# woolgathering/pyPeriod

Measured on AMD Instinct MI355X. Metric: window-projections/sec (all-p sweep, N=4096), higher is better.
Workload: dtype f64

## Files before the change

### include/periodhip.h

```cpp
#ifndef PERIODHIP_H
#define PERIODHIP_H

#include <stdint.h>

#ifdef __cplusplus
extern "C" {
#endif

#define PH_VERSION 100

#define PH_OK 0
#define PH_E_ARG (-1)
#define PH_E_HIP (-2)
#define PH_E_NOMEM (-3)
#define PH_E_CAP (-4)
#define PH_E_UNSUPPORTED (-5)

#define PH_F64 0
#define PH_F32 1

#define PH_FLAG_TRUNC 1u
#define PH_FLAG_ORTH 2u
#define PH_FLAG_SINGLE 4u
#define PH_FLAG_DEVICE 8u
// ... 9 lines not shown
#define PH_ST_NO_PERIOD 1
#define PH_ST_ITER_CAP 2
#define PH_ST_CAP 3

typedef struct ph_ctx ph_ctx;

int ph_version(void);
const char* ph_last_error(void);
int ph_device_count(int* count);
int ph_create(int device, ph_ctx** out);
int ph_destroy(ph_ctx* ctx);
#define PH_STREAM_DEFAULT ((void*)1)
int ph_set_stream(ph_ctx* ctx, void* hip_stream);
int ph_sync(ph_ctx* ctx);
int ph_timer_begin(ph_ctx* ctx);
int ph_timer_end(ph_ctx* ctx, float* elapsed_ms);
int ph_profile_enable(ph_ctx* ctx, int on);
int ph_profile_read(ph_ctx* ctx, float* ms, int cap, int* count);
const char* ph_profile_name(ph_ctx* ctx, int i);
int ph_device_info(ph_ctx* ctx, int* num_cu, int* lds_bytes);
int ph_max_window(ph_ctx* ctx, int dtype, unsigned flags, int* max_n);

int ph_sweep_plan_info(ph_ctx* ctx, int p_lo, int p_hi, int* n_pass, int* n_periods);

int ph_m_best_info(ph_ctx* ctx, int dtype, int N, int num, int min_length, int max_length, unsigned flags,
                   int* windows_per_workgroup, int* lds_bytes_per_sample);

int ph_m_best_plan_info(ph_ctx* ctx, int dtype, int N, int num, int min_length, int max_length, unsigned flags,
                        int* n_pass, int* n_periods);

int ph_m_best_screen_info(ph_ctx* ctx, int dtype, int N, int num, int min_length, int max_length, unsigned flags,
                          int gamma, int* n_entries, int* n_screened, long long* lds_elements);

int ph_periodic_norm(ph_ctx* ctx, const void* x, int dtype, int64_t W, int N, int p,
                     unsigned flags, double* out);

int ph_project_batch(ph_ctx* ctx, const void* x, int dtype, int64_t W, int N,
                     const int32_t* p_list, int n_p,
                     const int32_t* orth_off, const int32_t* orth_q, int table_max_p,
                     unsigned flags, void* out);

int ph_sweep(ph_ctx* ctx, const void* x, int dtype, int64_t W, int N, int p_lo, int p_hi,
             int mode, const int32_t* orth_off, const int32_t* orth_q, int table_max_p,
             unsigned flags, double* out);

int ph_m_best(ph_ctx* ctx, const void* x, int dtype, int64_t W, int N, int num,
// ... 136 lines not shown
```

### pyperiod_amd/_ffi.py

```python

from __future__ import annotations

import ctypes as C
import os

_HERE = os.path.dirname(os.path.abspath(__file__))
LIB_NAME = "libperiod_hip.so"
LIB_PATH = os.environ.get("PYPERIOD_AMD_LIB") or os.path.join(_HERE, LIB_NAME)

PH_OK, PH_E_ARG, PH_E_HIP, PH_E_NOMEM, PH_E_CAP, PH_E_UNSUPPORTED = 0, -1, -2, -3, -4, -5
PH_F64, PH_F32 = 0, 1
PH_FLAG_TRUNC, PH_FLAG_ORTH, PH_FLAG_SINGLE, PH_FLAG_DEVICE, PH_FLAG_NOSYNC = 1, 2, 4, 8, 16
PH_FLAG_KEEP_WEIGHTS = 32
PH_FLAG_OLA_NORM = 64
PH_STREAM_DEFAULT = 1
PH_SWEEP_NORM, PH_SWEEP_NORM_GAMMA, PH_SWEEP_MAXABS = 0, 1, 2
PH_ST_OK, PH_ST_NO_PERIOD, PH_ST_ITER_CAP, PH_ST_CAP = 0, 1, 2, 3
PH_QO_LDS_OVERLAY, PH_QO_LDS_BEHIND, PH_QO_HBM = 0, 1, 2
(PH_OP_PROJECT, PH_OP_SWEEP, PH_OP_M_BEST, PH_OP_SMALL_TO_LARGE, PH_OP_BEST_CORRELATION, PH_OP_BEST_FREQUENCY,
 PH_OP_RAMANUJAN, PH_OP_ORTH_POWERS, PH_OP_FOLD_SUMS, PH_OP_QO_FIT, PH_OP_QO_FIT_WIN, PH_OP_QO_ORTH_SELECT,
 PH_OP_QO_GET_PERIODS) = range(13)
PH_PLAN_KERNELS, PH_PLAN_K0, PH_PLAN_K1, PH_PLAN_STRIDE, PH_PLAN_LEN = 0, 1, 9, 8, 17
(PH_PLAN_VARIANT, PH_PLAN_WINDOW, PH_PLAN_SECOND, PH_PLAN_BLOCK, PH_PLAN_LDS_BYTES, PH_PLAN_SMALL_MEANS, PH_PLAN_WAVES,
 PH_PLAN_PAD) = range(8)
PH_PLAN_ONE, PH_PLAN_PAIR, PH_PLAN_FFT, PH_PLAN_CHIRP, PH_PLAN_DIRECT = 0, 1, 2, 3, 4
PH_PLAN_NONE, PH_PLAN_LDS, PH_PLAN_HBM = 0, 1, 2

_vp, _i, _i64, _u, _d = C.c_void_p, C.c_int, C.c_int64, C.c_uint, C.c_double
_pi32 = C.c_void_p

SIGNATURES = {
    "ph_version": [],
    "ph_device_count": [C.POINTER(_i)],
    "ph_create": [_i, C.POINTER(_vp)],
    "ph_destroy": [_vp],
    "ph_set_stream": [_vp, _vp],
    "ph_sync": [_vp],
    "ph_timer_begin": [_vp],
    "ph_timer_end": [_vp, C.POINTER(C.c_float)],
    "ph_device_info": [_vp, C.POINTER(_i), C.POINTER(_i)],
    "ph_max_window": [_vp, _i, _u, C.POINTER(_i)],
    "ph_sweep_plan_info": [_vp, _i, _i, C.POINTER(_i), C.POINTER(_i)],
    "ph_m_best_info": [_vp, _i, _i, _i, _i, _i, _u, C.POINTER(_i), C.POINTER(_i)],
    "ph_m_best_plan_info": [_vp, _i, _i, _i, _i, _i, _u, C.POINTER(_i), C.POINTER(_i)],
    "ph_m_best_screen_info": [_vp, _i, _i, _i, _i, _i, _u, _i, C.POINTER(_i), C.POINTER(_i), C.POINTER(C.c_longlong)],
    "ph_periodic_norm": [_vp, _vp, _i, _i64, _i, _i, _u, _vp],
    "ph_project_batch": [_vp, _vp, _i, _i64, _i, _pi32, _i, _pi32, _pi32, _i, _u, _vp],
    "ph_sweep": [_vp, _vp, _i, _i64, _i, _i, _i, _i, _pi32, _pi32, _i, _u, _vp],
    "ph_m_best": [_vp, _vp, _i, _i64, _i, _i, _i, _i, _i, _pi32, _pi32, _pi32, _pi32, _i, _u, _vp, _vp, _vp, _vp, _vp],
    "ph_profile_enable": [_vp, _i],
    "ph_profile_read": [_vp, C.POINTER(C.c_float), _i, C.POINTER(_i)],
    "ph_small_to_large": [_vp, _vp, _i, _i64, _i, _d, _i, _pi32, _pi32, _i, _u, _i, _vp, _vp, _vp, _vp, _vp],
    "ph_best_correlation": [_vp, _vp, _i, _i64, _i, _i, _i, _d, _pi32, _pi32, _i, _u, _vp, _vp, _vp, _vp],
    "ph_best_frequency": [_vp, _vp, _i, _i64, _i, _i, _i, _pi32, _pi32, _i, _u, _vp, _vp, _vp, _vp],
    "ph_ramanujan_norms": [_vp, _vp, _i, _i64, _i, _i, _i, _u, _vp],
    "ph_dict_project": [_vp, _vp, _vp, _i, _i, _u, _vp],
    "ph_qo_find_periods": [_vp, _vp, _i, _i64, _i, _i, _d, _i, _i, _i, _u, _vp, _vp, _vp, _vp, _vp, _vp, _vp],
    "ph_qo_greedy_win": [_vp, _vp, _i, _i64, _i, _vp, _i, _d, _i, _i, _i, _u, _vp, _vp, _vp, _vp, _vp, _vp, _vp],
    "ph_qo_fit": [_vp, _vp, _i, _i64, _i, _pi32, _pi32, _i, _i, _i, _i, _u, _vp, _vp, _vp, _vp],
    "ph_qo_fit_win": [_vp, _vp, _i, _i64, _i, _vp, _pi32, _pi32, _i, _i, _i, _i, _u, _vp, _vp, _vp, _vp],
    "ph_ramanujan_fit": [_vp, _vp, _i, _i64, _i, _i, _i, _d, _i, _i, _u, _vp, _vp, _vp, _vp, _vp, _vp, _vp],
    "ph_qo_feasible": [_vp, _i, _i, _i, _i, C.POINTER(_i)],
    "ph_qo_plan_info": [_vp, _i, _i, _i, _i, _u, C.POINTER(_i), C.POINTER(_i)],
    "ph_plan_info": [_vp, _i, _i, _i, _pi32, _i, _u, _pi32],
    "ph_orth_powers": [_vp, _vp, _i, _i64, _i, _i, _i, _u, _vp, _vp, _vp],
# ... 78 lines not shown
```

### pyperiod_amd/csrc/period_hip.hip

```cpp
#include <hip/hip_runtime.h>

#include <algorithm>
#include <cstdarg>
#include <cstdio>
#include <cstdlib>
#include <cstring>
#include <string>
#include <vector>

#include "../../include/periodhip.h"
#include "ph_kernels.h"
#include "ph_fit.h"
#include "ph_frames.h"

namespace {

thread_local std::string g_err;

int fail(int code, const char* fmt, ...) {
  char buf[512];
  va_list ap;
  va_start(ap, fmt);
  vsnprintf(buf, sizeof buf, fmt, ap);
  va_end(ap);
// ... 22 lines not shown

struct TableSlot {
  DevBuf dev;
  std::vector<int32_t> host;
  bool valid = false;
};

enum { T_PLIST, T_ORTH_OFF, T_ORTH_Q, T_FAC_OFF, T_FAC_Q, T_AUX0, T_AUX1, T_AUX2, T_AUX3, T_FIT_PHI, T_FIT_OFF, T_FIT_DQ, T_COUNT };
enum { B_IN, B_OUT0, B_OUT1, B_OUT2, B_OUT3, B_OUT4, B_WS0, B_WS1, B_GEN0, B_GBUF, B_GWIN, B_COUNT };

}

struct ph_ctx {
  int device = 0;
  hipStream_t own_stream = nullptr;
  hipStream_t stream = nullptr;
  hipEvent_t ev0 = nullptr, ev1 = nullptr;
  int num_cu = 0;
  int lds_limit = 0;
  DevBuf buf[B_COUNT];
  TableSlot tab[T_COUNT];
  DevBuf geom;
  DevBuf geomf;
  DevBuf kapf;
  int geom_n = -1, geom_max_p = -1;
  bool step1_pair = true;
  bool s2l_pair = true;
  bool bc_pair = true;
  bool pair_chain = true;
  bool pair_cover = true;
  bool pair_duo = true;
  DevBuf twid;
  int twid_len = -1;
  DevBuf bs_tab;
  int bs_L = -1, bs_M0 = -1;
  DevBuf plan;
  int plan_lo = -1, plan_hi = -1, plan_n = 0, plan_m = -1, plan_duo_n = 0;
  int plan_max_m = 4;
  int sweep_block = ph::kBlockWide;
  int step1_block = 0;
  int qo_block = 1024;
  int s2l_block = 1024;
  bool qo_hbm_window = false;
  bool hbm_window = false;
  int mob_max_p = -1;
  std::vector<int32_t> mob_off, mob_d, mob_mu;
// ... 110 lines not shown
  if (chains) max_m += 16;
  if (c->plan.p && c->plan_lo == p_lo && c->plan_hi == p_hi && c->plan_m == max_m && c->plan_duo_n == duo_n) {
    *out = static_cast<const ph::PassPlan*>(c->plan.p);
    *n_pass = c->plan_n;
    return PH_OK;
  }
  const std::vector<ph::PassPlan> host = build_plan(p_lo, p_hi, max_m & 7, mixed, chains, duo_n);
  PH_HIP(hipStreamSynchronize(c->stream));
  PH_TRY(ensure(c, c->plan, std::max<size_t>(1, host.size()) * sizeof(ph::PassPlan)));
  if (!host.empty())
    PH_HIP(hipMemcpyAsync(c->plan.p, host.data(), host.size() * sizeof(ph::PassPlan), hipMemcpyHostToDevice,
                          c->stream));
  PH_HIP(hipStreamSynchronize(c->stream));
  c->plan_lo = p_lo;
  c->plan_hi = p_hi;
  c->plan_m = max_m;
  c->plan_duo_n = duo_n;
  c->plan_n = (int)host.size();
  *out = static_cast<const ph::PassPlan*>(c->plan.p);
  *n_pass = c->plan_n;
  return PH_OK;
}

int prepare_geom(ph_ctx* c, int N, int max_p, const ph::PGeom** out) {
  if (c->geom.p && c->geom_n == N && c->geom_max_p >= max_p) {
    *out = static_cast<const ph::PGeom*>(c->geom.p);
    return PH_OK;
  }
  std::vector<ph::PGeom> host((size_t)max_p + 1);
  host[0] = ph::PGeom{0, 0, 0.0, 0.0};
  for (int p = 1; p <= max_p; ++p) {
    const int rows = (N + p - 1) / p;
    const int shortn = rows * p - N;
    host[p] = ph::PGeom{rows, p - shortn, 1.0 / rows, rows > 1 ? 1.0 / (rows - 1) : 0.0};
  }
  PH_HIP(hipStreamSynchronize(c->stream));
  PH_TRY(ensure(c, c->geom, host.size() * sizeof(ph::PGeom)));
  PH_HIP(hipMemcpyAsync(c->geom.p, host.data(), host.size() * sizeof(ph::PGeom), hipMemcpyHostToDevice, c->stream));
  std::vector<ph::PGeomF> hostf(host.size());
  for (size_t p = 0; p < host.size(); ++p)
    hostf[p] = ph::PGeomF{host[p].rows, host[p].nfull, (float)host[p].w_full, (float)host[p].w_short};
  PH_TRY(ensure(c, c->geomf, hostf.size() * sizeof(ph::PGeomF)));
  PH_HIP(hipMemcpyAsync(c->geomf.p, hostf.data(), hostf.size() * sizeof(ph::PGeomF), hipMemcpyHostToDevice, c->stream));
  std::vector<float> hostk(host.size(), 0.0f);
  for (size_t p = 1; p < host.size(); ++p) {
    const double k = ph::s2l_kappa(N, host[p].rows, (int)p);
    float f = (float)k;
    if ((double)f < k) f = std::nextafterf(f, INFINITY);
    hostk[p] = f;
  }
  PH_TRY(ensure(c, c->kapf, hostk.size() * sizeof(float)));
  PH_HIP(hipMemcpyAsync(c->kapf.p, hostk.data(), hostk.size() * sizeof(float), hipMemcpyHostToDevice, c->stream));
  PH_HIP(hipStreamSynchronize(c->stream));
  c->geom_n = N;
  c->geom_max_p = max_p;
  *out = static_cast<const ph::PGeom*>(c->geom.p);
  return PH_OK;
}

int check_common(ph_ctx* c, const void* x, int dtype, int64_t W, int N) {
  if (!c) return fail(PH_E_ARG, "ctx is NULL");
  if (!x) return fail(PH_E_ARG, "x is NULL");
  if (dtype != PH_F64 && dtype != PH_F32) return fail(PH_E_ARG, "dtype must be PH_F64 or PH_F32");
  if (W < 1 || W > 0x7fffffffLL / 64) return fail(PH_E_ARG, "W=%lld out of range", (long long)W);
  if (N < 1) return fail(PH_E_ARG, "N=%d must be >= 1", N);
  return PH_OK;
// ... 628 lines not shown
    if (v >= 64 && v <= 1024 && v % 64 == 0) c->qo_block = v;
  }
  if (std::getenv("PH_QO_HBM_WINDOW")) c->qo_hbm_window = true;
  if (const char* e = std::getenv("PH_HBM_WINDOW"))
    if (std::atoi(e) != 0) c->hbm_window = c->qo_hbm_window = true;
  if (const char* e = std::getenv("PH_SWEEP_BLOCK")) {
    const int v = std::atoi(e);
    if (v >= 64 && v <= 512 && v % 64 == 0) c->sweep_block = v;
  }
  *out = c;
  return PH_OK;
}

int ph_destroy(ph_ctx* c) {
  if (!c) return PH_OK;
  (void)hipSetDevice(c->device);
  (void)hipStreamSynchronize(c->stream);
  for (DevBuf& b : c->buf)
    if (b.p) (void)hipFree(b.p);
  for (TableSlot& t : c->tab)
    if (t.dev.p) (void)hipFree(t.dev.p);
  if (c->geom.p) (void)hipFree(c->geom.p);
  if (c->geomf.p) (void)hipFree(c->geomf.p);
  if (c->kapf.p) (void)hipFree(c->kapf.p);
  if (c->plan.p) (void)hipFree(c->plan.p);
  if (c->twid.p) (void)hipFree(c->twid.p);
  if (c->bs_tab.p) (void)hipFree(c->bs_tab.p);
  for (hipEvent_t e : c->prof_ev) (void)hipEventDestroy(e);
  if (c->ev0) (void)hipEventDestroy(c->ev0);
  if (c->ev1) (void)hipEventDestroy(c->ev1);
  if (c->own_stream) (void)hipStreamDestroy(c->own_stream);
  delete c;
  return PH_OK;
}

int ph_set_stream(ph_ctx* c, void* hip_stream) {
  if (!c) return fail(PH_E_ARG, "ctx is NULL");
  const hipError_t e = hipStreamSynchronize(c->stream);
  if (hip_stream == PH_STREAM_DEFAULT)
    c->stream = nullptr;
  else
    c->stream = hip_stream ? static_cast<hipStream_t>(hip_stream) : c->own_stream;
  if (e != hipSuccess) {
    (void)hipGetLastError();
    return fail(PH_E_HIP, "ph_set_stream: draining the previous stream failed (%s); the new stream is bound",
                hipGetErrorString(e));
  }
  return PH_OK;
}

int ph_sweep_plan_info(ph_ctx* c, int p_lo, int p_hi, int* n_pass, int* n_periods) {
  if (!c || !n_pass || !n_periods) return fail(PH_E_ARG, "NULL argument");
  if (p_lo < 1 || p_hi < p_lo) return fail(PH_E_ARG, "need 1 <= p_lo <= p_hi (got %d, %d)", p_lo, p_hi);
  *n_pass = (int)build_plan(p_lo, p_hi, c->plan_max_m, true, c->pair_chain).size();
  *n_periods = p_hi - p_lo + 1;
  return PH_OK;
}

int ph_m_best_info(ph_ctx* c, int dtype, int N, int num, int min_length, int max_length, unsigned flags,
                   int* windows_per_workgroup, int* lds_bytes_per_sample) {
  if (!c || !windows_per_workgroup || !lds_bytes_per_sample) return fail(PH_E_ARG, "NULL argument");
  if (dtype != PH_F64 && dtype != PH_F32) return fail(PH_E_ARG, "dtype must be PH_F64 or PH_F32");
  if (max_length < 0) max_length = N / 3;
  const bool pair = pair_eligible(c, dtype, N, num, min_length, max_length, flags);
  *windows_per_workgroup = pair ? 2 : 1;
  *lds_bytes_per_sample = pair ? 8 : (int)elem_size(dtype);
  return PH_OK;
}

int ph_m_best_plan_info(ph_ctx* c, int dtype, int N, int num, int min_length, int max_length, unsigned flags, int* n_pass,
                        int* n_periods) {
  if (!c || !n_pass || !n_periods) return fail(PH_E_ARG, "NULL argument");
  if (dtype != PH_F64 && dtype != PH_F32) return fail(PH_E_ARG, "dtype must be PH_F64 or PH_F32");
  if (max_length < 0) max_length = N / 3;
  if (min_length < 1 || max_length < min_length)
    return fail(PH_E_ARG, "need 1 <= min_length <= max_length (got %d, %d)", min_length, max_length);
  const bool pair = pair_eligible(c, dtype, N, num, min_length, max_length, flags);
  const int p_scr = pair ? pair_screen_lo(c, min_length, max_length, 0) : min_length;
// ... 352 lines not shown
  PH_TRY(st.in(x, (size_t)W * N * sz, &dx));
  PH_TRY(st.out(B_OUT0, periods, (size_t)W * num * sizeof(uint32_t), &dper));
  PH_TRY(st.out(B_OUT1, powers, (size_t)W * num * sizeof(double), &dpow));
  PH_TRY(st.out(B_OUT2, bases, (size_t)W * num * N * sz, &dbases));
  PH_TRY(st.out(B_OUT3, status, (size_t)W * sizeof(int32_t), &dstat));
  void* dsweeps;
  PH_TRY(st.out(B_OUT4, n_sweeps, (size_t)W * sizeof(int32_t), &dsweeps));
  PH_TRY(ensure(c, c->buf[B_WS0], (size_t)W * sizeof(double)));
  double* dnorm = static_cast<double*>(c->buf[B_WS0].p);
  const int row_stride = (max_length + 127) & ~127;
  PH_TRY(ensure(c, c->buf[B_WS1], (size_t)W * num * row_stride * sz));
  void* drows = c->buf[B_WS1].p;
  const unsigned kflags = flags & (PH_FLAG_TRUNC | PH_FLAG_ORTH);
  const int max_iters = 12 * (P + num) + 64;
  const dim3 grid((unsigned)W);
  if (pair) {
    const size_t gstride = ph::win_stride((size_t)N);
    PH_TRY(ensure(c, c->buf[B_GWIN], (size_t)W * gstride * sizeof(double)));
    auto kernel = ph::k_mbest_step1_pair;
    PH_TRY(allow_lds(kernel, s1.lds));
    ProfScope ps_(c, "k_mbest_step1");
    hipLaunchKernelGGL(kernel, dim3((unsigned)((W + 1) / 2)), dim3(s1.block), s1.lds, c->stream, (const double*)dx, (int)W, N,
                       num, min_length, max_length, p_scr, gamma, tb.fac_off, tb.fac_q, geom,
                       static_cast<const ph::PGeomF*>(c->geomf.p), plan, n_pass,
                       static_cast<double*>(c->buf[B_GWIN].p), max_iters, (uint32_t*)dper, (double*)dpow, (double*)drows,
                       row_stride, dnorm, (int*)dstat, (int*)dsweeps);
  } else
  PH_TRY(dispatch(dtype, !gwin1, [&](auto t, auto lw) {
    using T = decltype(t);
    auto kernel = ph::k_mbest_step1<T, decltype(lw)::value>;
    PH_TRY(allow_lds(kernel, s1.lds));
    ProfScope ps_(c, "k_mbest_step1");
    hipLaunchKernelGGL(kernel, grid, dim3(s1.block), s1.lds, c->stream, (const T*)dx, N, num, min_length,
                       max_length, gamma, kflags, tb, geom, plan, n_pass, (T*)gbuf1, (T*)gwin1, max_iters,
                       (uint32_t*)dper, (double*)dpow, (T*)drows, row_stride, dnorm, (int*)dstat, (int*)dsweeps, s1.small_means);
    return (int)PH_OK;
  }));
  PH_TRY(launch_check("k_mbest_step1"));
  PH_TRY(dispatch(dtype, !gwin2, [&](auto t, auto lw) {
    using T = decltype(t);
    auto kernel = ph::k_mbest_step2<T, decltype(lw)::value>;
    PH_TRY(allow_lds(kernel, s2.lds));
    ProfScope ps_(c, "k_mbest_step2");
    hipLaunchKernelGGL(kernel, grid, dim3(s2.block), s2.lds, c->stream, N, num, gamma,
                       max_length, kflags, tb, geom,
                       max_fac, (T*)gbuf2, (T*)gwin2, (uint32_t*)dper, (double*)dpow, (T*)dbases, dnorm,
                       (const int*)dstat, (T*)drows, row_stride);
// ... 1135 lines not shown
```

### pyperiod_amd/csrc/ph_device.h

```cpp
#pragma once

#include <hip/hip_runtime.h>
#include <stdint.h>

namespace ph {

constexpr int kWave = 64;
constexpr int kBlock = 256;
constexpr int kBlockWide = 512;
constexpr int kMaxWaves = 16;

constexpr unsigned kTrunc = 1u;
constexpr unsigned kOrth = 2u;
constexpr unsigned kSingle = 4u;

struct Tables {
  const int* orth_off;
  const int* orth_q;
  const int* fac_off;
  const int* fac_q;
};

typedef volatile __attribute__((address_space(3))) int* lds_int_ptr;

// ... 121 lines not shown

__device__ __forceinline__ double block_max(double v, double* red) {
  const int tid = threadIdx.x;
  const int nw = (blockDim.x + kWave - 1) / kWave;
  v = wave_max(v);
  if ((tid & (kWave - 1)) == 0) red[tid >> 6] = v;
  __syncthreads();
  const double t = red_combine<true>(red, nw);
  __syncthreads();
  return uniform_f64(t);
}

struct Fold {
  int p;
  int rows;
  int nfull;
  int trows;
  __device__ __forceinline__ Fold(int N, int p_) : p(p_) {
    rows = (N + p_ - 1) / p_;
    const int shortn = rows * p_ - N;
    nfull = p_ - shortn;
    trows = shortn == 0 ? rows : rows - 1;
  }
  __device__ __forceinline__ int count(int j) const { return j < nfull ? rows : rows - 1; }
};

template <typename T>
__device__ __forceinline__ T column_sum(const T* __restrict__ xs, int j, int p, int n) {
  if (n <= 0) return T(0);
  const T* ptr = xs + j;
  T s = ptr[0];
  ptr += p;
  int r = 1;
  for (; r + 8 <= n; r += 8) {
    T v[8];
#pragma unroll
    for (int u = 0; u < 8; ++u) v[u] = ptr[u * p];
#pragma unroll
    for (int u = 0; u < 8; ++u) s += v[u];
    ptr += 8 * p;
  }
  for (; r < n; ++r) {
    s += ptr[0];
    ptr += p;
  }
  return s;
// ... 720 lines not shown
```

### pyperiod_amd/csrc/ph_kernels.h

```cpp
#pragma once

#include <type_traits>

#include "ph_device.h"
#include "ph_pair.h"

namespace ph {

struct Carve {
  unsigned char* base;
  size_t off;
  __device__ explicit Carve(unsigned char* b) : base(b), off(0) {}
  template <typename U>
  __device__ U* take(size_t n) {
    U* p = reinterpret_cast<U*>(base + off);
    off += (n * sizeof(U) + 15) & ~size_t(15);
    return p;
  }
};

__host__ __device__ inline size_t carve_bytes(size_t n, size_t elem) { return (n * elem + 15) & ~size_t(15); }

__host__ __device__ inline size_t win_stride(size_t len) { return (len + 3) & ~size_t(3); }

// ... 322 lines not shown
__device__ __forceinline__ double pair_pick_scale(double rsq, int N) {
  if (!pair_usable(rsq)) return 1.0;
  int e;
  (void)frexp(rsq / (double)N, &e);
  return ldexp(1.0, -(e >> 1));
}

__device__ __forceinline__ int pair_rows_upper(float fn, int q) {
  return (int)(fn * __builtin_amdgcn_rcpf((float)q) * 1.000001f) + 1;
}

__device__ __forceinline__ double pair_exact_part(const double* __restrict__ xs, int p, const PGeom& g, int first, int stride) {
  double part = 0.0;
  for (int j = first; j < p; j += stride) {
    const bool full = j < g.nfull;
    const double s = column_sum(xs, j, p, full ? g.rows : g.rows - 1);
    part = fma(s * s, full ? g.w_full : g.w_short, part);
  }
  return part;
}

__global__ __launch_bounds__(1024) __attribute__((amdgpu_waves_per_eu(PH_STEP1_WAVES, 8))) void k_mbest_step1_pair(
    const double* __restrict__ x, int W, int N, int num, int p_lo, int p_hi, int p_scr, int gamma,
    const int* __restrict__ fac_off, const int* __restrict__ fac_q, const PGeom* __restrict__ geom, const PGeomF* __restrict__ geomf, const PassPlan* __restrict__ plan, int n_pass,
    double* __restrict__ gres, int max_iters, uint32_t* __restrict__ periods_out, double* __restrict__ norms_out,
    double* __restrict__ rows_out, int row_stride, double* __restrict__ dnorm_out, int* __restrict__ status_out,
    int* __restrict__ sweeps_out) {
  extern __shared__ __attribute__((aligned(16))) unsigned char smem[];
  Carve cv(smem);
  f2* pw = cv.take<f2>(N + kPad);
  double* stg = cv.take<double>(N + kPad);
  double* red = cv.take<double>(kRedDoubles);
  double* wbest = cv.take<double>(kMaxWaves);
  int* wbestp = cv.take<int>(kMaxWaves);
  double* norms = cv.take<double>(2 * num);
  uint32_t* periods = cv.take<uint32_t>(2 * num);
  const int P = p_hi - p_lo + 1;
  const int SK = (P + 31) / 32;
  uint32_t* skip = cv.take<uint32_t>(2 * SK);
  int* list = cv.take<int>(2 * kPairListCap);
  int* ctl = cv.take<int>(16);
  double* dst2 = cv.take<double>(4);
  double* msm = cv.take<double>(kPairSmallP);
  double* prt = cv.take<double>(kPairSplitW);

  const int tid = threadIdx.x;
  const int wv = __builtin_amdgcn_readfirstlane(tid >> 6);
// ... 27 lines not shown
      dst2[w] = rsq * sc * sc * (1.0 + 1e-9);
      dst2[2 + w] = sc;
      ctl[10 + w] = exists ? 1 : 0;
      ctl[12 + w] = pair_usable(rsq) ? 0 : 1;
      if (exists) dnorm_out[gw] = periodic_norm_from_sq_n(rsq, sqrtN, 0);
    }
  }
#ifdef PH_PAIR_TIMERS
#ifndef PH_PAIR_TIMERS_WGS
#define PH_PAIR_TIMERS_WGS 6
#endif
  long long ts[5] = {0, 0, 0, 0, 0};
  long long ts0 = wall_clock64();
  int nsurv_tot = 0, nall = 0;
#define PH_PAIR_MARK(k)                     \
  {                                         \
    const long long now_ = wall_clock64();  \
    ts[k] += now_ - ts0;                    \
    ts0 = now_;                             \
  }
#else
#define PH_PAIR_MARK(k)
#endif
  const float fn = (float)N;
#ifdef PH_CLOCKS
  const long long ck0 = clock64(), wk0 = wall_clock64();
#endif
  for (;;) {
    __syncthreads();
    const bool act0 = __builtin_amdgcn_readfirstlane(ctl[10]) != 0, act1 = __builtin_amdgcn_readfirstlane(ctl[11]) != 0;
    if (!act0 && !act1) break;
    prio_by_progress(__builtin_amdgcn_readfirstlane(max(ctl[8], ctl[9])));
    if (wv == 0 && pair_lane() == 0) ctl[0] = ctl[1] = 0;
    f2* vals = reinterpret_cast<f2*>(stg);
    pair_sweep_plan<false, true>(
        pw, N, geomf, plan, wv, n_pass, nw, [&](float z, int q) { pair_store1(vals, z, q, p_lo); },
        [&](float z, int q_a, int q_b) { pair_store2(vals, z, q_a, q_b, p_lo); },
        PH_PAIR_QUEUE ? &ctl[14] : nullptr);
    __syncthreads();
    PH_PAIR_MARK(0)
    prio_short_phase();
    {
    const int tid = (wv << 6) + pair_lane();
    const int lane = tid & (kWave - 1);
    if (tid == 0) ctl[14] = nw;
    {
      const bool scr0 = act0 && !__builtin_amdgcn_readfirstlane(ctl[12]), scr1 = act1 && !__builtin_amdgcn_readfirstlane(ctl[13]);
      if (scr0 || scr1) {
        const double unit0 = uniform_f64(dst2[0]), unit1 = uniform_f64(dst2[1]);
        const int i0 = p_scr - p_lo;
        const bool cover = i0 > 0;
        const int SD = (i0 + 31) >> 5;
        uint32_t* seen = reinterpret_cast<uint32_t*>(stg);
        for (int k = tid; k < 2 * SD; k += blockDim.x) seen[k] = 0u;
        const double slack = cover ? pair_cover_slack(N) : 0.0;
        double lo0 = -1.0 / 0.0, lo1 = -1.0 / 0.0;
        for (int idx = i0 + tid; idx < P; idx += blockDim.x) {
          const int q = p_lo + idx;
          const f2 v = vals[idx];
          const double rad = pair_radius(pair_rows_upper(fn, q), q);
          const uint32_t bit = 1u << (idx & 31);
          double a = (double)v.x - rad * unit0, b = (double)v.y - rad * unit1;
          if (gamma) {
            const double rq = 1.0 / (double)q;
            a *= rq;
            b *= rq;
          }
          if (!(skip[idx >> 5] & bit) && a > lo0) lo0 = a;
          if (!(skip[SK + (idx >> 5)] & bit) && b > lo1) lo1 = b;
        }
        lo0 = wave_max(lo0);
        lo1 = wave_max(lo1);
        if (lane == 0) {
          red[wv] = lo0;
          red[kMaxWaves + wv] = lo1;
        }
        __syncthreads();
        lo0 = uniform_f64(red_combine<true>(red, nw));
        lo1 = uniform_f64(red_combine<true>(red + kMaxWaves, nw));
        const bool none0 = cover && scr0 && !(lo0 > -1.0 / 0.0), none1 = cover && scr1 && !(lo1 > -1.0 / 0.0);
        if (tid == 0 && none0) ctl[0] = kPairListCap + 1;
        if (tid == 0 && none1) ctl[1] = kPairListCap + 1;
        const double thr0 = lo0 - fabs(lo0) * 1e-9, thr1 = lo1 - fabs(lo1) * 1e-9;
        for (int idx = i0 + tid; idx < P; idx += blockDim.x) {
          const int q = p_lo + idx;
          const f2 v = vals[idx];
          const double rad = pair_radius(pair_rows_upper(fn, q), q) + slack;
          const uint32_t bit = 1u << (idx & 31);
          double a = (double)v.x + rad * unit0, b = (double)v.y + rad * unit1;
          if (gamma) {
            const double rq = 1.0 / (double)q;
            a *= rq;
            b *= rq;
          }
          const bool hit0 = scr0 && !none0 && a >= thr0, hit1 = scr1 && !none1 && b >= thr1;
          if (hit0 && !(skip[idx >> 5] & bit)) {
            const int k = atomicAdd(&ctl[0], 1);
            if (k < kPairListCap) list[k] = q;
          }
          if (hit1 && !(skip[SK + (idx >> 5)] & bit)) {
            const int k = atomicAdd(&ctl[1], 1);
            if (k < kPairListCap) list[kPairListCap + k] = q;
          }
          if (cover && (hit0 || hit1)) {
            const int f1 = fac_off[q + 1];
            for (int f = fac_off[q] - (p_lo == 1 ? 1 : 0); f < f1; ++f) {
              const int d = f < fac_off[q] ? 1 : fac_q[f];
              if (d < p_lo || d >= p_scr) continue;
              const int di = d - p_lo;
              const uint32_t dbit = 1u << (di & 31);
              for (int w = 0; w < 2; ++w) {
                if (!(w ? hit1 : hit0) || (skip[w * SK + (di >> 5)] & dbit)) continue;
                if (atomicOr(&seen[w * SD + (di >> 5)], dbit) & dbit) continue;
                const int k = atomicAdd(&ctl[w], 1);
                if (k < kPairListCap) list[w * kPairListCap + k] = d;
              }
            }
          }
        }
      }
    }
    __syncthreads();
    PH_PAIR_MARK(1)
// ... 88 lines not shown
        } else {
          for (int k = wv; k < ncand; k += nw) {
            const int p = exact_all ? p_lo + k : lst[k];
            if ((sk[(p - p_lo) >> 5] >> ((p - p_lo) & 31)) & 1u) continue;
            const PGeom g = geom[p];
            const double part = p < 64 ? wave_partial_small(stg, N, p, g, lane) : pair_exact_part(stg, p, g, lane, kWave);
            consider(wave_sum(part), p);
          }
          best = bestp != 0 ? periodic_norm_from_sq_n(best_ss, sqrtN, gamma ? bestp : 0) : 0.0;
          if (!(best > 0.0)) bestp = 0;
          if (lane == 0) {
            wbest[wv] = best;
            wbestp[wv] = bestp;
          }
          __syncthreads();
          red_argmax(wbest, wbestp, nw, best, bestp);
          __syncthreads();
        }
        PH_PAIR_MARK(3)
        if (bestp == 0) {
          status = 1;
        } else {
          int row = -1;
          for (int k = 0; k < num; ++k)
            if (per[k] == (uint32_t)bestp) row = k;
          int action;
          __syncthreads();
          if (row >= 0 && repeats < 10) {
            action = 2;
            if (tid == 0) nrm[row] += best;
            repeats += 1;
          } else if (row >= 0) {
            action = 0;
            if (tid == 0) sk[(bestp - p_lo) >> 5] |= 1u << ((bestp - p_lo) & 31);
            repeats = 0;
          } else {
            action = 1;
            row = filled;
            if (tid == 0) {
              per[row] = (uint32_t)bestp;
              nrm[row] = best;
            }
            filled += 1;
            repeats = 0;
          }
          double* brow = rows_out + (gw * (int64_t)num + (row < 0 ? 0 : row)) * row_stride;
          const bool more = filled < num;
          const double sc = uniform_f64(dst2[2 + w]);
          double* dst = gres + gw * gstride;
          double acc = 0.0;
          const Fold f(N, bestp);
          if (bestp <= kPairSmallP) {
            split_row_means(stg, msm, prt, N, bestp, tid, kPairSplitW);
            if (tid < bestp) {
              const double m = msm[tid];
              if (action == 1)
                brow[tid] = m;
              else if (action == 2)
                brow[tid] += m;
            }
            if (more) {
              int idx = tid % bestp;
              const int step = blockDim.x % bestp;
              for (int n = tid; n < N; n += blockDim.x) {
                const double v = stg[n] - msm[idx];
                dst[n] = v;
                pwf[2 * n + w] = (float)(v * sc);
                acc = fma(v, v, acc);
                idx += step;
                idx = idx >= bestp ? idx - bestp : idx;
              }
            }
          } else {
            for (int j = tid; j < bestp; j += blockDim.x) {
// ... 2395 lines not shown
```

### pyperiod_amd/csrc/ph_pair.h

```cpp
#pragma once

#include "ph_device.h"

namespace ph {

typedef float f2 __attribute__((ext_vector_type(2)));
typedef const volatile __attribute__((address_space(3))) f2* pair_ptr;

struct PGeomF {
  int rows;
  int nfull;
  float w_full;
  float w_short;
};

__device__ __forceinline__ f2 f2_make(float a, float b) {
  f2 r;
  r.x = a;
  r.y = b;
  return r;
}
__device__ __forceinline__ f2 f2_zero() { return f2_make(0.0f, 0.0f); }
__device__ __forceinline__ f2 f2_fma(f2 a, f2 b, f2 c) { return __builtin_elementwise_fma(a, b, c); }
__device__ __forceinline__ f2 f2_max(f2 a, f2 b) { return __builtin_elementwise_max(a, b); }
// ... 241 lines not shown
      "v_pk_fma_f32 %[acc], %[v], %[v], %[acc]\n\t"
      "s_mov_b64 exec, %[keep]"
      : [acc] "+v"(acc), [keep] "=&s"(keep)
      : [v] "v"(v), [m] "s"(lanes)
      : "scc");
}
__device__ __forceinline__ void f2_sq_acc_cut(f2& sa, f2& pa, f2& sb, f2& pb, f2 t, f2 d, unsigned long below, unsigned long inq) {
  unsigned long keep;
  asm volatile(
      "s_and_saveexec_b64 %[keep], %[below]\n\t"
      "v_pk_fma_f32 %[sa], %[t], %[t], %[sa]\n\t"
      "v_pk_fma_f32 %[pa], %[d], %[d], %[pa]\n\t"
      "s_andn2_b64 exec, %[keep], %[below]\n\t"
      "v_pk_fma_f32 %[pb], %[d], %[d], %[pb]\n\t"
      "s_and_b64 exec, exec, %[inq]\n\t"
      "v_pk_fma_f32 %[sb], %[t], %[t], %[sb]\n\t"
      "s_mov_b64 exec, %[keep]"
      : [sa] "+v"(sa), [pa] "+v"(pa), [sb] "+v"(sb), [pb] "+v"(pb), [keep] "=&s"(keep)
      : [t] "v"(t), [d] "v"(d), [below] "s"(below), [inq] "s"(inq)
      : "scc");
}

template <int R, int NR, int U, int PRO>
__device__ __forceinline__ void pair_duo_group(pair_ptr ptr, int q, int c, f2 (&pend)[R - 1], f2& sa, f2& pa, f2& sb, f2& pb) {
  static_assert(NR == R || NR == R - 1, "all rows (in front of the cut), or all but the last (behind it)");
  static_assert(PRO >= -1 && PRO <= U, "columns without a square are columns of the group");
  f2 v[NR][U];
#pragma unroll
  for (int r = 0; r < NR; ++r)
#pragma unroll
    for (int u = 0; u < U; ++u) v[r][u] = ptr[r * q + 64 * u];
  __builtin_amdgcn_s_waitcnt(0xC07F);
  __builtin_amdgcn_sched_barrier(0);
#pragma unroll
  for (int u = 0; u < U; ++u) {
    f2 t = v[0][u];
#pragma unroll
    for (int r = 1; r < NR; ++r) t += v[r][u];
    if (NR == R) sa = f2_fma(t, t, sa);
    else sb = f2_fma(t, t, sb);
    if (u >= PRO) {
      f2 d = pend[R - 2];
      if (NR == R) d += v[NR - 1][u];
      if (PRO < 0) d *= scalar_select_lt(c + u, R - 1, 0.0f, 1.0f);
      if (NR == R) pa = f2_fma(d, d, pa);
      else pb = f2_fma(d, d, pb);
    }
#pragma unroll
    for (int k = R - 2; k >= 1; --k) pend[k] = pend[k - 1] + v[k][u];
    pend[0] = v[0][u];
  }
}

template <int R, int NR>
__device__ __forceinline__ void pair_duo_edge(pair_ptr ptr, int q, unsigned long below, unsigned long inq, f2 (&pend)[R - 1],
                                              f2& sa, f2& pa, f2& sb, f2& pb) {
  static_assert(NR == R || NR == R - 1, "all rows (in front of the cut), or all but the last (behind it)");
  f2 v[NR];
#pragma unroll
  for (int r = 0; r < NR; ++r) v[r] = ptr[r * q];
  __builtin_amdgcn_s_waitcnt(0xC07F);
  __builtin_amdgcn_sched_barrier(0);
  f2 t = v[0];
#pragma unroll
  for (int r = 1; r < NR; ++r) t += v[r];
  f2 d = pend[R - 2];
  if (NR == R) d += v[NR - 1];
// ... 8 lines not shown
  pend[0] = v[0];
}

template <int R, int T0, int T1>
__device__ __forceinline__ void pair_duo_tail(const f2* __restrict__ xs, int q, int ncb, f2 (&pend)[R - 1], f2& pb) {
  const pair_ptr at = pair_at(xs) + 64 * ncb;
  f2 v[R - 1][R - 1];
#pragma unroll
  for (int t = T0; t < T1; ++t)
#pragma unroll
    for (int r = t; r < R - 1; ++r) v[r][t] = at[r * q + 64 * t];
  __builtin_amdgcn_s_waitcnt(0xC07F);
  __builtin_amdgcn_sched_barrier(0);
#pragma unroll
  for (int t = T0; t < T1; ++t) {
    pb = f2_fma(pend[R - 2], pend[R - 2], pb);
#pragma unroll
    for (int k = R - 2; k >= 1; --k) pend[k] = k >= t ? pend[k - 1] + v[k][t] : pend[k - 1];
    if (t == 0) pend[0] = v[0][0];
  }
  if (T1 == R - 1) f2_sq_acc_lanes(pb, pend[R - 2], pair_lanes_below(q - 64 * (ncb - 1)));
}

template <int R>
__device__ __forceinline__ void pair_duo_rows(const f2* __restrict__ xs, int N, int q, const PGeomF g, f2& base, f2& partner) {
  constexpr int UA = R <= 4 ? 4 : 2, UB = R <= 4 ? 4 : R == 5 ? 3 : 2;
  constexpr int A3 = UA < 4 ? 1 : 3, A2 = UA < 3 ? 1 : 2, B3 = UB < 4 ? 1 : 3, B2 = UB < 3 ? 1 : 2;
  constexpr int P0 = R - 1 < UA ? R - 1 : UA, P1 = R - 1 - UA < UA ? R - 1 - UA : UA, P2 = R - 1 - 2 * UA;
  const int cut = g.nfull, ncb = (q + 63) >> 6, last = ncb - 1;
  f2 pend[R - 1];
#pragma unroll
  for (int k = 0; k < R - 1; ++k) pend[k] = f2_zero();
  f2 sa = f2_zero(), pa = f2_zero(), sb, pb;
  int c = 0;
  {
    const int whole = min(cut >> 6, last);
    const pair_ptr at = pair_at(xs);
    if (UA <= whole) {
      pair_duo_group<R, R, UA, P0>(at, q, 0, pend, sa, pa, sb, pb);
      c = UA;
      if constexpr (P1 > 0) {
        if (2 * UA <= whole) {
          pair_duo_group<R, R, UA, P1>(at + 64 * UA, q, UA, pend, sa, pa, sb, pb);
          c = 2 * UA;
          if constexpr (P2 > 0) {
            if (3 * UA <= whole) {
              pair_duo_group<R, R, UA, P2>(at + 128 * UA, q, 2 * UA, pend, sa, pa, sb, pb);
              c = 3 * UA;
            }
          }
        }
      }
    }
    for (; c + UA <= whole; c += UA) pair_duo_group<R, R, UA, 0>(at + 64 * c, q, c, pend, sa, pa, sb, pb);
    const int rem = whole - c;
    if (rem > 0) {
      asm volatile("" ::: "memory");
      if (c < R - 1) {
        if (UA > 3 && rem == 3) pair_duo_group<R, R, A3, -1>(at + 64 * c, q, c, pend, sa, pa, sb, pb);
        else if (UA > 2 && rem == 2) pair_duo_group<R, R, A2, -1>(at + 64 * c, q, c, pend, sa, pa, sb, pb);
        else pair_duo_group<R, R, 1, -1>(at + 64 * c, q, c, pend, sa, pa, sb, pb);
      } else {
        if (UA > 3 && rem == 3) pair_duo_group<R, R, A3, 0>(at + 64 * c, q, c, pend, sa, pa, sb, pb);
        else if (UA > 2 && rem == 2) pair_duo_group<R, R, A2, 0>(at + 64 * c, q, c, pend, sa, pa, sb, pb);
        else pair_duo_group<R, R, 1, 0>(at + 64 * c, q, c, pend, sa, pa, sb, pb);
      }
      c = whole;
    }
  }
  sb = pb = f2_zero();
  const unsigned long inq = pair_lanes_below(q - 64 * last);
  if (c < last && 64 * c < cut) {
    asm volatile("" ::: "memory");
    pair_duo_edge<R, R>(pair_at(xs) + 64 * c, q, pair_lanes_below(cut - 64 * c), ~0ul, pend, sa, pa, sb, pb);
    c += 1;
  }
  {
    const pair_ptr at = pair_at(xs);
    for (; c + UB <= last; c += UB) pair_duo_group<R, R - 1, UB, 0>(at + 64 * c, q, c, pend, sa, pa, sb, pb);
    const int rem = last - c;
    if (rem > 0) {
      asm volatile("" ::: "memory");
      if (UB > 3 && rem == 3) pair_duo_group<R, R - 1, B3, 0>(at + 64 * c, q, c, pend, sa, pa, sb, pb);
      else if (UB > 2 && rem == 2) pair_duo_group<R, R - 1, B2, 0>(at + 64 * c, q, c, pend, sa, pa, sb, pb);
      else pair_duo_group<R, R - 1, 1, 0>(at + 64 * c, q, c, pend, sa, pa, sb, pb);
    }
  }
  asm volatile("" ::: "memory");
  if (64 * last < cut) pair_duo_edge<R, R>(pair_at(xs) + 64 * last, q, pair_lanes_below(cut - 64 * last), inq, pend, sa, pa, sb, pb);
  else pair_duo_edge<R, R - 1>(pair_at(xs) + 64 * last, q, 0ul, inq, pend, sa, pa, sb, pb);
  const f2 wf = f2_make(g.w_full, g.w_full);
  base = f2_fma(sa, wf, sb * g.w_short);
  if (R == 6) {
    pair_duo_tail<R, 0, 2>(xs, q, ncb, pend, pb);
    pair_duo_tail<R, 2, R - 1>(xs, q, ncb, pend, pb);
  } else {
    pair_duo_tail<R, 0, R - 1>(xs, q, ncb, pend, pb);
  }
  partner = f2_fma(pa, wf, pb * g.w_short);
}

__device__ __forceinline__ void pair_pass_duo(const f2* __restrict__ xs, int N, int q, const PGeomF g, f2& base, f2& partner) {
  base = partner = f2_zero();
  switch (g.rows) {
#define PH_DUO_CASE(R)                                \
  case R:                                             \
    pair_duo_rows<R>(xs, N, q, g, base, partner);     \
    break;
// ... 202 lines not shown
      pair_chain_small<MX>(xs, N, p, m - 8, geom, consume, consume2);
    } else if (m == 0) {
      consume(red(pair_partial_small<MX>(xs, N, p, geom[p])), p);
    } else if (m == 1) {
      consume(red(pair_pass_single<MX>(xs, p, geom[p])), p);
    } else if (DUO && m == 3) {
      f2 va, vb;
      pair_pass_duo(xs, N, p, geom[p], va, vb);
      consume2(pair_reduce2<MX>(va, vb), p, p + 64);
    } else if (m == 2) {
      f2 part[3];
      pair_pass_multi<2, MX>(xs, p, geom, part);
      consume2(pair_reduce2<MX>(part[0], part[1]), p, 2 * p);
    } else {
      f2 part[3];
      pair_pass_multi<4, MX>(xs, p, geom, part);
      consume2(pair_reduce2<MX>(part[0], part[1]), p, 2 * p);
      consume(red(part[2]), 4 * p);
    }
    i = queue ? lds_ticket_value(ticket) : i + stride;
  }
}

__device__ __forceinline__ double pair_radius(int rows, int q) {
  return 1.5 * (2.0 * (double)rows + (double)(q >> 6) + 32.0) * 5.9604644775390625e-08;
}

__device__ __forceinline__ double pair_cover_slack(int N) {
  return fmax(9.094947017729282e-13, (2.0 * (double)N + 32.0) * 2.220446049250313e-16);
}

}
```

Before: 9.549 billion.

## Precompute pair radius table, peel duo remainder first, unroll loops, ballot row search

```diff
diff --git a/include/periodhip.h b/include/periodhip.h
--- a/include/periodhip.h
+++ b/include/periodhip.h
@@ -55,6 +55,8 @@
 int ph_max_window(ph_ctx* ctx, int dtype, unsigned flags, int* max_n);
 
 int ph_sweep_plan_info(ph_ctx* ctx, int p_lo, int p_hi, int* n_pass, int* n_periods);
+
+int ph_pair_radius_table(int N, int max_p, double* out);
 
 int ph_m_best_info(ph_ctx* ctx, int dtype, int N, int num, int min_length, int max_length, unsigned flags,
                    int* windows_per_workgroup, int* lds_bytes_per_sample);
diff --git a/pyperiod_amd/_ffi.py b/pyperiod_amd/_ffi.py
--- a/pyperiod_amd/_ffi.py
+++ b/pyperiod_amd/_ffi.py
@@ -41,6 +41,7 @@
     "ph_device_info": [_vp, C.POINTER(_i), C.POINTER(_i)],
     "ph_max_window": [_vp, _i, _u, C.POINTER(_i)],
     "ph_sweep_plan_info": [_vp, _i, _i, C.POINTER(_i), C.POINTER(_i)],
+    "ph_pair_radius_table": [_i, _i, C.POINTER(_d)],
     "ph_m_best_info": [_vp, _i, _i, _i, _i, _i, _u, C.POINTER(_i), C.POINTER(_i)],
     "ph_m_best_plan_info": [_vp, _i, _i, _i, _i, _i, _u, C.POINTER(_i), C.POINTER(_i)],
     "ph_m_best_screen_info": [_vp, _i, _i, _i, _i, _i, _u, _i, C.POINTER(_i), C.POINTER(_i), C.POINTER(C.c_longlong)],
diff --git a/pyperiod_amd/csrc/period_hip.hip b/pyperiod_amd/csrc/period_hip.hip
--- a/pyperiod_amd/csrc/period_hip.hip
+++ b/pyperiod_amd/csrc/period_hip.hip
@@ -68,6 +68,7 @@
   TableSlot tab[T_COUNT];
   DevBuf geom;
   DevBuf geomf;
+  DevBuf radq;
   DevBuf kapf;
   int geom_n = -1, geom_max_p = -1;
   bool step1_pair = true;
@@ -224,6 +225,12 @@
   return PH_OK;
 }
 
+std::vector<double> pair_radius_table(int N, int max_p) {
+  std::vector<double> host((size_t)max_p + 1, 0.0);
+  for (int q = 1; q <= max_p; ++q) host[q] = ph::pair_radius((N + q - 1) / q, q);
+  return host;
+}
+
 int prepare_geom(ph_ctx* c, int N, int max_p, const ph::PGeom** out) {
   if (c->geom.p && c->geom_n == N && c->geom_max_p >= max_p) {
     *out = static_cast<const ph::PGeom*>(c->geom.p);
@@ -244,6 +251,9 @@
     hostf[p] = ph::PGeomF{host[p].rows, host[p].nfull, (float)host[p].w_full, (float)host[p].w_short};
   PH_TRY(ensure(c, c->geomf, hostf.size() * sizeof(ph::PGeomF)));
   PH_HIP(hipMemcpyAsync(c->geomf.p, hostf.data(), hostf.size() * sizeof(ph::PGeomF), hipMemcpyHostToDevice, c->stream));
+  const std::vector<double> hostr = pair_radius_table(N, max_p);
+  PH_TRY(ensure(c, c->radq, hostr.size() * sizeof(double)));
+  PH_HIP(hipMemcpyAsync(c->radq.p, hostr.data(), hostr.size() * sizeof(double), hipMemcpyHostToDevice, c->stream));
   std::vector<float> hostk(host.size(), 0.0f);
   for (size_t p = 1; p < host.size(); ++p) {
     const double k = ph::s2l_kappa(N, host[p].rows, (int)p);
@@ -918,6 +928,7 @@
     if (t.dev.p) (void)hipFree(t.dev.p);
   if (c->geom.p) (void)hipFree(c->geom.p);
   if (c->geomf.p) (void)hipFree(c->geomf.p);
+  if (c->radq.p) (void)hipFree(c->radq.p);
   if (c->kapf.p) (void)hipFree(c->kapf.p);
   if (c->plan.p) (void)hipFree(c->plan.p);
   if (c->twid.p) (void)hipFree(c->twid.p);
@@ -950,6 +961,14 @@
   if (p_lo < 1 || p_hi < p_lo) return fail(PH_E_ARG, "need 1 <= p_lo <= p_hi (got %d, %d)", p_lo, p_hi);
   *n_pass = (int)build_plan(p_lo, p_hi, c->plan_max_m, true, c->pair_chain).size();
   *n_periods = p_hi - p_lo + 1;
+  return PH_OK;
+}
+
+int ph_pair_radius_table(int N, int max_p, double* out) {
+  if (!out) return fail(PH_E_ARG, "NULL argument");
+  if (N < 1 || max_p < 1 || max_p > N) return fail(PH_E_ARG, "need 1 <= max_p <= N (got %d, %d)", max_p, N);
+  const std::vector<double> host = pair_radius_table(N, max_p);
+  std::copy(host.begin(), host.end(), out);
   return PH_OK;
 }
 
@@ -1348,7 +1367,7 @@
     ProfScope ps_(c, "k_mbest_step1");
     hipLaunchKernelGGL(kernel, dim3((unsigned)((W + 1) / 2)), dim3(s1.block), s1.lds, c->stream, (const double*)dx, (int)W, N,
                        num, min_length, max_length, p_scr, gamma, tb.fac_off, tb.fac_q, geom,
-                       static_cast<const ph::PGeomF*>(c->geomf.p), plan, n_pass,
+                       static_cast<const ph::PGeomF*>(c->geomf.p), static_cast<const double*>(c->radq.p), plan, n_pass,
                        static_cast<double*>(c->buf[B_GWIN].p), max_iters, (uint32_t*)dper, (double*)dpow, (double*)drows,
                        row_stride, dnorm, (int*)dstat, (int*)dsweeps);
   } else
diff --git a/pyperiod_amd/csrc/ph_device.h b/pyperiod_amd/csrc/ph_device.h
--- a/pyperiod_amd/csrc/ph_device.h
+++ b/pyperiod_amd/csrc/ph_device.h
@@ -167,6 +167,7 @@
     nfull = p_ - shortn;
     trows = shortn == 0 ? rows : rows - 1;
   }
+  __device__ __forceinline__ Fold(int p_, int rows_, int nfull_) : p(p_), rows(rows_), nfull(nfull_), trows(nfull_ == p_ ? rows_ : rows_ - 1) {}
   __device__ __forceinline__ int count(int j) const { return j < nfull ? rows : rows - 1; }
 };
 
diff --git a/pyperiod_amd/csrc/ph_kernels.h b/pyperiod_amd/csrc/ph_kernels.h
--- a/pyperiod_amd/csrc/ph_kernels.h
+++ b/pyperiod_amd/csrc/ph_kernels.h
@@ -368,7 +368,7 @@
 
 __global__ __launch_bounds__(1024) __attribute__((amdgpu_waves_per_eu(PH_STEP1_WAVES, 8))) void k_mbest_step1_pair(
     const double* __restrict__ x, int W, int N, int num, int p_lo, int p_hi, int p_scr, int gamma,
-    const int* __restrict__ fac_off, const int* __restrict__ fac_q, const PGeom* __restrict__ geom, const PGeomF* __restrict__ geomf, const PassPlan* __restrict__ plan, int n_pass,
+    const int* __restrict__ fac_off, const int* __restrict__ fac_q, const PGeom* __restrict__ geom, const PGeomF* __restrict__ geomf, const double* __restrict__ radq, const PassPlan* __restrict__ plan, int n_pass,
     double* __restrict__ gres, int max_iters, uint32_t* __restrict__ periods_out, double* __restrict__ norms_out,
     double* __restrict__ rows_out, int row_stride, double* __restrict__ dnorm_out, int* __restrict__ status_out,
     int* __restrict__ sweeps_out) {
@@ -442,7 +442,6 @@
 #else
 #define PH_PAIR_MARK(k)
 #endif
-  const float fn = (float)N;
 #ifdef PH_CLOCKS
   const long long ck0 = clock64(), wk0 = wall_clock64();
 #endif
@@ -474,20 +473,35 @@
         uint32_t* seen = reinterpret_cast<uint32_t*>(stg);
         for (int k = tid; k < 2 * SD; k += blockDim.x) seen[k] = 0u;
         const double slack = cover ? pair_cover_slack(N) : 0.0;
+        struct Entry {
+          f2 v;
+          double rad, rq;
+          bool skip0, skip1;
+        };
+        auto entry = [&](int idx) {
+          Entry e;
+          const int q = p_lo + idx;
+          const uint32_t bit = 1u << (idx & 31);
+          e.v = vals[idx];
+          e.rad = radq[q];
+          e.rq = gamma ? 1.0 / (double)q : 1.0;
+          e.skip0 = (skip[idx >> 5] & bit) != 0;
+          e.skip1 = (skip[SK + (idx >> 5)] & bit) != 0;
+          return e;
+        };
+        const int idx_own = i0 + tid;
+        Entry own = {f2_zero(), 0.0, 1.0, true, true};
+        if (idx_own < P) own = entry(idx_own);
         double lo0 = -1.0 / 0.0, lo1 = -1.0 / 0.0;
-        for (int idx = i0 + tid; idx < P; idx += blockDim.x) {
-          const int q = p_lo + idx;
-          const f2 v = vals[idx];
-          const double rad = pair_radius(pair_rows_upper(fn, q), q);
-          const uint32_t bit = 1u << (idx & 31);
-          double a = (double)v.x - rad * unit0, b = (double)v.y - rad * unit1;
+        for (int idx = idx_own; idx < P; idx += blockDim.x) {
+          const Entry e = idx == idx_own ? own : entry(idx);
+          double a = (double)e.v.x - e.rad * unit0, b = (double)e.v.y - e.rad * unit1;
           if (gamma) {
-            const double rq = 1.0 / (double)q;
-            a *= rq;
-            b *= rq;
-          }
-          if (!(skip[idx >> 5] & bit) && a > lo0) lo0 = a;
-          if (!(skip[SK + (idx >> 5)] & bit) && b > lo1) lo1 = b;
+            a *= e.rq;
+            b *= e.rq;
+          }
+          if (!e.skip0 && a > lo0) lo0 = a;
+          if (!e.skip1 && b > lo1) lo1 = b;
         }
         lo0 = wave_max(lo0);
         lo1 = wave_max(lo1);
@@ -502,23 +516,21 @@
         if (tid == 0 && none0) ctl[0] = kPairListCap + 1;
         if (tid == 0 && none1) ctl[1] = kPairListCap + 1;
         const double thr0 = lo0 - fabs(lo0) * 1e-9, thr1 = lo1 - fabs(lo1) * 1e-9;
-        for (int idx = i0 + tid; idx < P; idx += blockDim.x) {
+        for (int idx = idx_own; idx < P; idx += blockDim.x) {
+          const Entry e = idx == idx_own ? own : entry(idx);
           const int q = p_lo + idx;
-          const f2 v = vals[idx];
-          const double rad = pair_radius(pair_rows_upper(fn, q), q) + slack;
-          const uint32_t bit = 1u << (idx & 31);
-          double a = (double)v.x + rad * unit0, b = (double)v.y + rad * unit1;
+          const double rad = e.rad + slack;
+          double a = (double)e.v.x + rad * unit0, b = (double)e.v.y + rad * unit1;
           if (gamma) {
-            const double rq = 1.0 / (double)q;
-            a *= rq;
-            b *= rq;
+            a *= e.rq;
+            b *= e.rq;
           }
           const bool hit0 = scr0 && !none0 && a >= thr0, hit1 = scr1 && !none1 && b >= thr1;
-          if (hit0 && !(skip[idx >> 5] & bit)) {
+          if (hit0 && !e.skip0) {
             const int k = atomicAdd(&ctl[0], 1);
             if (k < kPairListCap) list[k] = q;
           }
-          if (hit1 && !(skip[SK + (idx >> 5)] & bit)) {
+          if (hit1 && !e.skip1) {
             const int k = atomicAdd(&ctl[1], 1);
             if (k < kPairListCap) list[kPairListCap + k] = q;
           }
@@ -653,8 +665,10 @@
           status = 1;
         } else {
           int row = -1;
-          for (int k = 0; k < num; ++k)
-            if (per[k] == (uint32_t)bestp) row = k;
+          for (int k0 = 0; k0 < num; k0 += kWave) {
+            const unsigned long long hit = __ballot(k0 + lane < num && per[k0 + lane] == (uint32_t)bestp);
+            if (hit) row = k0 + 63 - __clzll(hit);
+          }
           int action;
           __syncthreads();
           if (row >= 0 && repeats < 10) {
@@ -680,7 +694,8 @@
           const double sc = uniform_f64(dst2[2 + w]);
           double* dst = gres + gw * gstride;
           double acc = 0.0;
-          const Fold f(N, bestp);
+          const PGeom gb = geom[__builtin_amdgcn_readfirstlane(bestp)];
+          const Fold f(bestp, gb.rows, gb.nfull);
           if (bestp <= kPairSmallP) {
             split_row_means(stg, msm, prt, N, bestp, tid, kPairSplitW);
             if (tid < bestp) {
diff --git a/pyperiod_amd/csrc/ph_pair.h b/pyperiod_amd/csrc/ph_pair.h
--- a/pyperiod_amd/csrc/ph_pair.h
+++ b/pyperiod_amd/csrc/ph_pair.h
@@ -287,9 +287,9 @@
 }
 
 template <int R, int NR, int U, int PRO>
-__device__ __forceinline__ void pair_duo_group(pair_ptr ptr, int q, int c, f2 (&pend)[R - 1], f2& sa, f2& pa, f2& sb, f2& pb) {
+__device__ __forceinline__ void pair_duo_group(pair_ptr ptr, int q, f2 (&pend)[R - 1], f2& sa, f2& pa, f2& sb, f2& pb) {
   static_assert(NR == R || NR == R - 1, "all rows (in front of the cut), or all but the last (behind it)");
-  static_assert(PRO >= -1 && PRO <= U, "columns without a square are columns of the group");
+  static_assert(PRO >= 0 && PRO <= U, "columns without a square are columns of the group");
   f2 v[NR][U];
 #pragma unroll
   for (int r = 0; r < NR; ++r)
@@ -307,7 +307,6 @@
     if (u >= PRO) {
       f2 d = pend[R - 2];
       if (NR == R) d += v[NR - 1][u];
-      if (PRO < 0) d *= scalar_select_lt(c + u, R - 1, 0.0f, 1.0f);
       if (NR == R) pa = f2_fma(d, d, pa);
       else pb = f2_fma(d, d, pb);
     }
@@ -362,51 +361,46 @@
   if (T1 == R - 1) f2_sq_acc_lanes(pb, pend[R - 2], pair_lanes_below(q - 64 * (ncb - 1)));
 }
 
+template <int R, int UA, int S>
+__device__ __forceinline__ void pair_duo_peel(pair_ptr at, int q, f2 (&pend)[R - 1], f2& sa, f2& pa, f2& sb, f2& pb) {
+  if constexpr (S < R - 1) {
+    pair_duo_group<R, R, UA, (R - 1 - S < UA ? R - 1 - S : UA)>(at + 64 * S, q, pend, sa, pa, sb, pb);
+    pair_duo_peel<R, UA, S + UA>(at, q, pend, sa, pa, sb, pb);
+  }
+}
+template <int R, int UA, int F>
+__device__ __forceinline__ int pair_duo_front(pair_ptr at, int q, f2 (&pend)[R - 1], f2& sa, f2& pa, f2& sb, f2& pb) {
+  static_assert(F >= 1 && F <= UA, "the first group is the remainder, or a full group");
+  pair_duo_group<R, R, F, (R - 1 < F ? R - 1 : F)>(at, q, pend, sa, pa, sb, pb);
+  pair_duo_peel<R, UA, F>(at, q, pend, sa, pa, sb, pb);
+  return F >= R - 1 ? F : F + (R - 1 - F + UA - 1) / UA * UA;
+}
+
 template <int R>
 __device__ __forceinline__ void pair_duo_rows(const f2* __restrict__ xs, int N, int q, const PGeomF g, f2& base, f2& partner) {
   constexpr int UA = R <= 4 ? 4 : 2, UB = R <= 4 ? 4 : R == 5 ? 3 : 2;
-  constexpr int A3 = UA < 4 ? 1 : 3, A2 = UA < 3 ? 1 : 2, B3 = UB < 4 ? 1 : 3, B2 = UB < 3 ? 1 : 2;
-  constexpr int P0 = R - 1 < UA ? R - 1 : UA, P1 = R - 1 - UA < UA ? R - 1 - UA : UA, P2 = R - 1 - 2 * UA;
+  constexpr int B3 = UB < 4 ? 1 : 3, B2 = UB < 3 ? 1 : 2;
   const int cut = g.nfull, ncb = (q + 63) >> 6, last = ncb - 1;
   f2 pend[R - 1];
 #pragma unroll
   for (int k = 0; k < R - 1; ++k) pend[k] = f2_zero();
   f2 sa = f2_zero(), pa = f2_zero(), sb, pb;
-  int c = 0;
+  int c;
   {
     const int whole = min(cut >> 6, last);
     const pair_ptr at = pair_at(xs);
-    if (UA <= whole) {
-      pair_duo_group<R, R, UA, P0>(at, q, 0, pend, sa, pa, sb, pb);
-      c = UA;
-      if constexpr (P1 > 0) {
-        if (2 * UA <= whole) {
-          pair_duo_group<R, R, UA, P1>(at + 64 * UA, q, UA, pend, sa, pa, sb, pb);
-          c = 2 * UA;
-          if constexpr (P2 > 0) {
-            if (3 * UA <= whole) {
-              pair_duo_group<R, R, UA, P2>(at + 128 * UA, q, 2 * UA, pend, sa, pa, sb, pb);
-              c = 3 * UA;
-            }
-          }
-        }
+    const int rem = whole & (UA - 1);
+    if (UA > 3 && rem == 3) c = pair_duo_front<R, UA, (UA > 3 ? 3 : 1)>(at, q, pend, sa, pa, sb, pb);
+    else if (UA > 2 && rem == 2) c = pair_duo_front<R, UA, (UA > 2 ? 2 : 1)>(at, q, pend, sa, pa, sb, pb);
+    else if (rem == 1) c = pair_duo_front<R, UA, 1>(at, q, pend, sa, pa, sb, pb);
+    else c = pair_duo_front<R, UA, UA>(at, q, pend, sa, pa, sb, pb);
+    if constexpr (R <= 4) {
+      for (; c + 2 * UA <= whole; c += 2 * UA) {
+        pair_duo_group<R, R, UA, 0>(at + 64 * c, q, pend, sa, pa, sb, pb);
+        pair_duo_group<R, R, UA, 0>(at + 64 * c + 64 * UA, q, pend, sa, pa, sb, pb);
       }
     }
-    for (; c + UA <= whole; c += UA) pair_duo_group<R, R, UA, 0>(at + 64 * c, q, c, pend, sa, pa, sb, pb);
-    const int rem = whole - c;
-    if (rem > 0) {
-      asm volatile("" ::: "memory");
-      if (c < R - 1) {
-        if (UA > 3 && rem == 3) pair_duo_group<R, R, A3, -1>(at + 64 * c, q, c, pend, sa, pa, sb, pb);
-        else if (UA > 2 && rem == 2) pair_duo_group<R, R, A2, -1>(at + 64 * c, q, c, pend, sa, pa, sb, pb);
-        else pair_duo_group<R, R, 1, -1>(at + 64 * c, q, c, pend, sa, pa, sb, pb);
-      } else {
-        if (UA > 3 && rem == 3) pair_duo_group<R, R, A3, 0>(at + 64 * c, q, c, pend, sa, pa, sb, pb);
-        else if (UA > 2 && rem == 2) pair_duo_group<R, R, A2, 0>(at + 64 * c, q, c, pend, sa, pa, sb, pb);
-        else pair_duo_group<R, R, 1, 0>(at + 64 * c, q, c, pend, sa, pa, sb, pb);
-      }
-      c = whole;
-    }
+    for (; c + UA <= whole; c += UA) pair_duo_group<R, R, UA, 0>(at + 64 * c, q, pend, sa, pa, sb, pb);
   }
   sb = pb = f2_zero();
   const unsigned long inq = pair_lanes_below(q - 64 * last);
@@ -417,13 +411,17 @@
   }
   {
     const pair_ptr at = pair_at(xs);
-    for (; c + UB <= last; c += UB) pair_duo_group<R, R - 1, UB, 0>(at + 64 * c, q, c, pend, sa, pa, sb, pb);
+    for (; c + 2 * UB <= last; c += 2 * UB) {
+      pair_duo_group<R, R - 1, UB, 0>(at + 64 * c, q, pend, sa, pa, sb, pb);
+      pair_duo_group<R, R - 1, UB, 0>(at + 64 * c + 64 * UB, q, pend, sa, pa, sb, pb);
+    }
+    for (; c + UB <= last; c += UB) pair_duo_group<R, R - 1, UB, 0>(at + 64 * c, q, pend, sa, pa, sb, pb);
     const int rem = last - c;
     if (rem > 0) {
       asm volatile("" ::: "memory");
-      if (UB > 3 && rem == 3) pair_duo_group<R, R - 1, B3, 0>(at + 64 * c, q, c, pend, sa, pa, sb, pb);
-      else if (UB > 2 && rem == 2) pair_duo_group<R, R - 1, B2, 0>(at + 64 * c, q, c, pend, sa, pa, sb, pb);
-      else pair_duo_group<R, R - 1, 1, 0>(at + 64 * c, q, c, pend, sa, pa, sb, pb);
+      if (UB > 3 && rem == 3) pair_duo_group<R, R - 1, B3, 0>(at + 64 * c, q, pend, sa, pa, sb, pb);
+      else if (UB > 2 && rem == 2) pair_duo_group<R, R - 1, B2, 0>(at + 64 * c, q, pend, sa, pa, sb, pb);
+      else pair_duo_group<R, R - 1, 1, 0>(at + 64 * c, q, pend, sa, pa, sb, pb);
     }
   }
   asm volatile("" ::: "memory");
@@ -672,7 +670,7 @@
   }
 }
 
-__device__ __forceinline__ double pair_radius(int rows, int q) {
+__host__ __device__ __forceinline__ double pair_radius(int rows, int q) {
   return 1.5 * (2.0 * (double)rows + (double)(q >> 6) + 32.0) * 5.9604644775390625e-08;
 }
 
```

Measured after the change: 9.725 billion, median of 6. +1.8%, better.
